# showlab/DiffSim

Measured on AMD Instinct MI355X. Metric: image-pairs/sec at 512px, SD1.5 up_blocks[0] t=600, higher is better.
Workload: dtype bf16

## Files before the change

### diffsim_amd/csrc/common.h

```cpp
#pragma once
#include <hip/hip_runtime.h>
#include <stddef.h>
#include <stdint.h>

#include "../../include/diffsim_amd.h"

namespace dsim {

typedef __bf16 bf16_t;
typedef _Float16 f16_t;
#ifdef DSIM_H16_IS_F16
typedef _Float16 h16;
#define DSIM_H16_NS f16
#define DSIM_H16 DSIM_F16
#define DSIM_H16_ONE_BITS 0x3C00u
#define DSIM_H16_LSUM_MAX 3.0e4f
#define H16_MFMA_16x16x32 __builtin_amdgcn_mfma_f32_16x16x32_f16
#define H16_MFMA_32x32x16 __builtin_amdgcn_mfma_f32_32x32x16_f16
#else
typedef __bf16 h16;
#define DSIM_H16_NS bf16
#define DSIM_H16 DSIM_BF16
#define DSIM_H16_ONE_BITS 0x3F80u
#define DSIM_H16_LSUM_MAX 1e30f
#define H16_MFMA_16x16x32 __builtin_amdgcn_mfma_f32_16x16x32_bf16
#define H16_MFMA_32x32x16 __builtin_amdgcn_mfma_f32_32x32x16_bf16
#endif
typedef __attribute__((ext_vector_type(8))) h16 h16x8;
typedef __attribute__((ext_vector_type(4))) h16 h16x4;
typedef __attribute__((ext_vector_type(2))) h16 h16x2;
typedef __attribute__((ext_vector_type(4))) float f32x4;
typedef __attribute__((ext_vector_type(16))) float f32x16;
typedef __attribute__((ext_vector_type(4))) unsigned int u32x4;
typedef __attribute__((ext_vector_type(2))) unsigned int u32x2;

#ifdef __HIPCC__
__device__ __forceinline__ h16x4 h16_ds_read_tr16_b64(const char* p) {
#ifdef DSIM_H16_IS_F16
    typedef __fp16 fp16v4 __attribute__((__vector_size__(4 * sizeof(__fp16))));
    return __builtin_bit_cast(h16x4, __builtin_amdgcn_ds_read_tr16_b64_v4f16((__attribute__((address_space(3))) fp16v4*)(p)));
#else
    return __builtin_amdgcn_ds_read_tr16_b64_v4bf16((__attribute__((address_space(3))) h16x4*)(p));
#endif
}
__device__ __forceinline__ float gelu_fast(float x) {
    const float u = fminf(x * x, 64.0f);
    const float t = x * fmaf(u, fmaf(u, 1.01426306e-3f, -0.106775724f), -2.30112134f);
    return x * __builtin_amdgcn_rcpf(1.0f + __builtin_amdgcn_exp2f(t));
}
__device__ __forceinline__ float max_halves(float x) {
    const unsigned u = __float_as_uint(x);
    const auto r = __builtin_amdgcn_permlane32_swap(u, u, false, false);
    return fmaxf(__uint_as_float(r[0]), __uint_as_float(r[1]));
}
__device__ __forceinline__ float half_sum(float x) {
    const unsigned u = __float_as_uint(x);
    const auto r = __builtin_amdgcn_permlane32_swap(u, u, false, false);
    return __uint_as_float(r[0]) + __uint_as_float(r[1]);
}
constexpr unsigned BUF_OOB = 0x80000000u;
__device__ __forceinline__ __attribute__((const)) __amdgpu_buffer_rsrc_t buf_rsrc(const void* ptr, unsigned bytes) {
    return __builtin_amdgcn_make_buffer_rsrc((void*)ptr, 0, (int)bytes, 0x00020000);
}
#endif

#define DSIM_HIP_CHECK(expr)                                   \
    do {                                                       \
        hipError_t _e = (expr);                                \
        if (_e != hipSuccess) return DSIM_ERR_HIP;             \
    } while (0)

static inline size_t dtype_size(int dt) { return dt == DSIM_F32 ? 4 : 2; }
static inline const char* dtype_name(int dt) { return dt == DSIM_F32 ? "f32" : (dt == DSIM_F16 ? "f16" : "bf16"); }

template <typename T> struct Elem { typedef T type; };
template <typename F>
int by_dtype(int dtype, F&& f) {
    switch (dtype) {
        case DSIM_BF16: return f(Elem<bf16_t>{});
        case DSIM_F16: return f(Elem<f16_t>{});
        case DSIM_F32: return f(Elem<float>{});
    }
    return DSIM_ERR_INVALID;
}
template <typename F, typename Twin>
int by_h16_dtype(int dtype, F&& f, Twin&& twin) {
    if (dtype == DSIM_H16) return f(Elem<h16>{});
#ifndef DSIM_H16_IS_F16
    if (dtype == DSIM_F32) return f(Elem<float>{});
    if (dtype == DSIM_F16) return twin();
#endif
    return DSIM_ERR_INVALID;
}

static inline size_t up256(size_t bytes) { return (bytes + 255) & ~(size_t)255; }

enum GemmMode { GEMM_LINEAR = 0, GEMM_CONV3 = 1, GEMM_CONV3P = 2 };
enum GemmEpi { EPI_NONE = 0, EPI_RESIDUAL = 1, EPI_GEGLU = 2 };
enum { EK_PLAIN = 0, EK_RES = 1, EK_SLOW = 2, EK_ACT = 3,
       EK_PLAIN_GN = 4, EK_RES_GN = 5 };

struct GemmArgs {
    const void* A0 = nullptr;
    const void* A1 = nullptr;
    int C0 = 0, C1 = 0;
    int mode = GEMM_LINEAR;
    int Hin = 0, Win = 0, Hout = 0, Wout = 0;
    int stride = 1, ups = 0;
    int pad = 1;
    int lwo = -1, lhw = -1;
    int M = 0, N = 0, K = 0;
    const void* W = nullptr;
    const float* bias = nullptr;
    const float* bias2 = nullptr;
    int rows_per_batch = 0;
    int act = 0;
    const float* gate = nullptr;
    const float* gate2 = nullptr;
    int epi = EPI_NONE;
    int geglu_blk = 32;
    const void* residual = nullptr;
    void* out = nullptr;
    int ldo = 0;
    int out_split = 0;
    long long out_split_stride = 0;
    int force_big = 0;
    int wb_rows = 0;
    unsigned wb_stride = 0;
    float* gn_part = nullptr;
    int gn_hw = 0;
    const void* zero_page = nullptr;
    unsigned a0_bytes = 0, a1_bytes = 0, w_bytes = 0, out_bytes = 0;
#ifdef DSIM_DEVTOOLS
    int exp = 0;
    unsigned long long* stamps = nullptr;
#endif
};
struct GemmLaunchRec {
    int bm = 0, bn = 0, mode = -1, geglu = 0, ek = -1, small = 0;
};
extern thread_local GemmLaunchRec g_gemm_last_launch;
inline int geglu_block_rows(int N) { return (N % 320 == 0 && N != 8 * 320) ? 16 : 32; }
#ifdef DSIM_DEVTOOLS
extern int g_gemm_persistent;
extern int g_force_bm;
extern int g_gemm_exp;
extern int g_gemm_skinny;
extern unsigned long long* g_gemm_stamps;
extern int g_skinny_tile;
extern int g_attn_dbg;
extern float* g_tail160_dbg;
extern int g_tail160_exp;
extern int g_ff_dbg;
extern int g_rl_dbg;
extern int g_rl_wpc;
extern int g_ff_stagger;
#else
constexpr int g_gemm_skinny = 1, g_gemm_persistent = 1, g_force_bm = 0, g_gemm_exp = 0, g_skinny_tile = 0;
constexpr int g_rl_wpc = 3, g_ff_stagger = -1;
#endif
constexpr int kSkinnyTiles[][2] = {{64, 64}, {64, 80}, {64, 128}, {128, 80}, {128, 128},
#ifdef DSIM_DEVTOOLS
                                   {128, 64}, {128, 160},
#endif
};
constexpr int kSkinnyChoices = 5, kSkinnyCompiled = sizeof(kSkinnyTiles) / sizeof(kSkinnyTiles[0]);
int pack_linear(const void* src, int src_dtype, void* dst, int dst_dtype, int N, int K,
                int geglu_interleave, hipStream_t s);
int pack_conv3(const void* src, int src_dtype, void* dst, int dst_dtype, int Cout, int Cin,
               hipStream_t s);
int pack_conv_in(const void* src, int src_dtype, float* dst, int Cout, int Cin, hipStream_t s);
int pack_vector(const void* src, int src_dtype, float* dst, int N, int geglu_interleave,
                hipStream_t s);
int gemv_f32(const void* W, int w_dtype, const void* bias, int b_dtype, const float* x, float* y,
             int N, int K, int act, hipStream_t s);
int add_vectors_f32(const float* a, const float* b, float* out, int N, hipStream_t s);
int timestep_sincos(float* out, int dim, int t, hipStream_t s);
int sincos_values(float* out, int dim, const float* vals , int count, hipStream_t s);

int prep_conv_in(const float* lat, const float* noise , float sa, float sb, const float* w ,
                 const float* bias, void* out, int dtype, int n_img, int Cin, int S, int Cout, int dup ,
                 hipStream_t st);
enum { CONV_IN_GENERIC = 1, CONV_IN_EIGHT = 2, CONV_IN_ROWS = 3 };
bool prep_conv_in_kind_applies(int kind, int Cin, int Cout);
int prep_conv_in_kind(int Cin, int Cout);
int prep_conv_in_as(int kind, const float* lat, const float* noise, float sa, float sb, const float* w, const float* bias, void* out,
                    int dtype, int n_img, int Cin, int S, int Cout, int dup, hipStream_t st);
bool conv_in_rows_applies(int Cin, int S, int Cout);
int conv_in_rows(const float* images, const float* w , const float* bias, void* out, int dtype, int n_img, int S,
                 float* gn_part, hipStream_t st);
int convert_f32_to(const float* src, void* dst, int dtype, size_t n, hipStream_t s);
int gather_ctx(const float* ctx, int n_ctx, const int32_t* index, void* dst, int dtype, int n_images, size_t per, hipStream_t s);
int dup_batch(const void* in, void* out, int n_batch, size_t bytes_per_elem, hipStream_t s);
int resize_nearest(const void* in, void* out, int B, int Hin, int Win, int Hout, int Wout, size_t row_bytes, hipStream_t s);

int patch_embed(const float* lat, const float* noise, float sa, float sb, const float* w, const float* bias, const float* pos, void* out,
                int dtype, int n_img, int Cin, int S, int p, int D, hipStream_t s);
int fold_quant(const float* wq, const void* wco, const float* bco, const float* bq, void* out_w, float* out_b, int Cm, int K, int dtype,
               hipStream_t s);
int to_nchw_f32(const void* x, float* out, int n, int HW, int C, int dtype, hipStream_t s);

struct RowLinArgs {
    const void* x = nullptr;
    void* out = nullptr;
    const float* ln_g = nullptr;
    const float* ln_b = nullptr;
    const void* stream = nullptr;
    int M = 0, C = 0, N = 0;
    float eps = 1e-5f;
    int dtype = DSIM_BF16;
    int gn = 0;
    const float* coef = nullptr;
    const float* bias = nullptr;
    int HW = 0;
};

int image_preprocess(const unsigned char* hwc, float* out, int n, int H, int W, int half, hipStream_t s);
int latent_sample(const float* moments, const float* eps, float* out, int n_out, int first, int stride, int C, int hw, int eps_n,
                  float sf, int round16, hipStream_t s);

size_t groupnorm_scratch_bytes(int B, int groups);
int groupnorm_passes(int C0, int C1, int HW, int groups, int dtype);
int groupnorm_plan(int C0, int C1, int B, int HW, int groups, int dtype, int pre, dsim_gn_plan* plan);
int layernorm_plan(int M, int C, int dtype, int mod, dsim_ln_plan* plan);
int launch_groupnorm(const void* x0, int C0, const void* x1, int C1, const float* gamma,
                     const float* beta, void* out, int B, int HW, int groups, float eps, int silu,
                     int dtype, void* scratch, hipStream_t s);
int launch_groupnorm_pre(const void* x, int C, const float* gamma, const float* beta, void* out, int B, int HW, int groups, float eps,
                         int silu, int dtype, void* scratch, const float* part32, int chunks, hipStream_t s);
int launch_groupnorm_stats(const void* x, int C, const float* gamma, const float* beta, int B, int HW, int groups, float eps, int dtype,
                           void* scratch, float* coef, hipStream_t s);
int launch_layernorm(const void* x, const float* gamma, const float* beta, void* out, int M, int C,
                     float eps, int dtype, hipStream_t s);
int launch_layernorm_mod(const void* x, const float* scale2, const float* shift2, void* out, int M, int C,
                         int rows_per_batch, float eps, int dtype, hipStream_t s);
int launch_softmax_rows(const void* x, void* out, int rows, int cols, float scale, int dtype, hipStream_t s);

struct AttnArgs {
    const void* q = nullptr; int ldq = 0;
    const void* k = nullptr; const void* v = nullptr; int ldk = 0;
    void* out = nullptr; int ldo = 0;
    int B = 0, Bkv = 0, H = 0, Nq = 0, Nk = 0, D = 0;
    int xcd_remap = 1;
};
enum class AttnKernel {
    P160 = DSIM_ATTN_P160,
    Short = DSIM_ATTN_SHORT,
    ShortK80 = DSIM_ATTN_SHORT_K80,
    Long = DSIM_ATTN_LONG,
    Q2 = DSIM_ATTN_Q2,
    Q2Fast = DSIM_ATTN_Q2FAST,
    Fast = DSIM_ATTN_FAST,
    Exact = DSIM_ATTN_EXACT,
};
inline const char* attn_kind_suffix(int kind) {
    switch (kind) {
        case DSIM_ATTN_P160: return "_p160";
        case DSIM_ATTN_SHORT:
        case DSIM_ATTN_SHORT_K80: return "_short";
        case DSIM_ATTN_LONG: return "_long";
        case DSIM_ATTN_Q2: return "_q2";
        case DSIM_ATTN_Q2FAST: return "_q2fast";
        case DSIM_ATTN_FAST: return "_fast";
        default: return "";
    }
}
struct AttnLaunchRec {
    int kind = -1, D = 0, dtype = -1, k80 = 0, qit = 0, grid = 0;
};
extern thread_local AttnLaunchRec g_attn_last_launch;
int launch_attention_fp8(const AttnArgs& a, hipStream_t s);

struct PairArgs {
    const void* q = nullptr;
    const void* k = nullptr;
    const void* v = nullptr;
    const int32_t* idx_a = nullptr;
    const int32_t* idx_b = nullptr;
    int n_pairs = 0, B = 0, H = 0, N = 0, D = 0;
    int similarity = 0;
    void* scratch = nullptr;
    size_t scratch_bytes = 0;
};

struct MatrixArgs {
    const void* q[2];
    const void* k[2];
    const void* v[2];
    const uint8_t* mask[2];
    int n_a, n_b, B, H, N, D;
    int similarity;
    void* scratch;
    size_t scratch_bytes;
};

struct FFArgs {
    const void* x = nullptr;
    void* out = nullptr;
    const float* ln_g = nullptr;
    const float* ln_b = nullptr;
    const void* stream = nullptr;
    const float* b1 = nullptr;
    const float* b2 = nullptr;
    int M = 0, C = 0;
    float eps = 1e-5f;
    int dtype = DSIM_BF16;
};

inline namespace DSIM_H16_NS {
#include "h16_api.h"
inline bool gemm_gn_stats_tile(const GemmArgs& a, int dtype) {
    if (dtype == DSIM_F32 || a.mode != GEMM_CONV3 || a.epi == EPI_GEGLU || a.bias2 || a.Wout <= 0) return false;
    const int hw = a.Hout * a.Wout;
    if ((a.Wout & (a.Wout - 1)) || (hw & (hw - 1)) || hw % 256) return false;
    float asked = 0.f;
    GemmArgs q = a;
    q.gn_part = &asked; q.gn_hw = hw; q.zero_page = &asked;
    GemmLaunchRec plan;
    return gemm_plan(q, dtype, &plan) == DSIM_OK;
}
inline int pair_args_check(const PairArgs& a, int dtype, bool tiled = true) {
    if (dtype != DSIM_F32 && dtype != DSIM_BF16 && dtype != DSIM_F16) return DSIM_ERR_INVALID;
    if (a.similarity != 0 && a.similarity != 1) return DSIM_ERR_INVALID;
    return pair_shape_served(a.n_pairs, a.B, a.H, a.N, a.D, tiled) ? DSIM_OK : DSIM_ERR_INVALID;
}
inline int matrix_args_check(const MatrixArgs& a, int dtype, bool listed) {
    if (a.similarity != 0 && a.similarity != 1) return DSIM_ERR_INVALID;
    return matrix_shape_served(a.n_a, a.n_b, a.B, a.H, a.N, a.D, dtype, listed) ? DSIM_OK : DSIM_ERR_INVALID;
}
}
#if !defined(DSIM_H16_IS_F16) && !defined(DSIM_DEVTOOLS)
namespace f16 {
#include "h16_api.h"
}
#define DSIM_F16_TWIN(call) f16::call
#else
#define DSIM_F16_TWIN(call) DSIM_ERR_INVALID
#endif

int cu_count();
struct DeviceOnce {
    unsigned long long done = 0;
    template <typename F> int ensure(F&& apply) {
        int dev = 0;
        if (hipGetDevice(&dev) != hipSuccess) return DSIM_ERR_HIP;
        if (dev >= 0 && dev < 64 && (__atomic_load_n(&done, __ATOMIC_ACQUIRE) >> dev) & 1ull) return DSIM_OK;
        const int st = apply();
        if (st == DSIM_OK && dev >= 0 && dev < 64) __atomic_fetch_or(&done, 1ull << dev, __ATOMIC_RELEASE);
        return st;
    }
};
template <auto Kern, typename... A>
int launch_lds(dim3 grid, dim3 block, int lds_bytes, hipStream_t s, A... args) {
    static DeviceOnce once;
    const int st = once.ensure([&]() -> int {
        return hipFuncSetAttribute((const void*)Kern, hipFuncAttributeMaxDynamicSharedMemorySize, lds_bytes) == hipSuccess ? DSIM_OK
                                                                                                                            : DSIM_ERR_HIP;
    });
    if (st != DSIM_OK) return st;
    hipLaunchKernelGGL(Kern, grid, block, lds_bytes, s, args...);
    return hipGetLastError() == hipSuccess ? DSIM_OK : DSIM_ERR_HIP;
}

}
```

### diffsim_amd/csrc/rowres.hip

```cpp
#include "common.h"

namespace dsim {
namespace {

constexpr int RC = 320;
constexpr int RKS = RC / 16;
constexpr int RNB = RC / 32;
constexpr int RNCH = 4 * RC / 32;
constexpr int RITER = RNCH + 2;
constexpr int RW1B = 64 * RC * 2;
constexpr int RW2B = RC * 64;
constexpr int RCHB = RW1B + RW2B;
constexpr int RPIECES = RCHB / 1024;
constexpr int RPW = RPIECES / 4;
constexpr int RB1 = 0, RB2 = 8 * RC, RLG = 9 * RC, RLB = 10 * RC, RVEC = 11 * RC;
constexpr int SLABP = 144;
constexpr int RSCR = 32 * SLABP;
constexpr int RLDS = 2 * RCHB + RVEC * 4 + 4 * RSCR;
static_assert(RPIECES % 4 == 0 && RITER % 2 == 0, "ring geometry");

__device__ __forceinline__ int slab_chunk(int row, int cpos) { return cpos ^ ((row >> 1) & 7); }
__device__ __forceinline__ int slab_off(int row, int c) { const int s = (row >> 1) & 7; return row * 128 + ((c ^ s) << 4); }
__device__ __forceinline__ u32x4 slab_image(const h16* __restrict__ w, int row0, int slab, int row, int cpos, int ldw = RC, int k0 = 0) {
    const int cl = slab_chunk(row, cpos);
    return *reinterpret_cast<const u32x4*>(w + (size_t)(row0 + row) * ldw + k0 + 64 * slab + 8 * cl);
}

__global__ void pack_ff_stream_kernel(const h16* __restrict__ w1p, const h16* __restrict__ w2p, char* __restrict__ stream) {
    const int i = blockIdx.x * blockDim.x + threadIdx.x;
    if (i >= RITER * (RCHB / 16)) return;
    const int ci = i / (RCHB / 16), o = (i - ci * (RCHB / 16)) * 16;
    u32x4 v = {0u, 0u, 0u, 0u};
    if (o < RW1B) {
        if (ci < RNCH) v = slab_image(w1p, 64 * ci, o / 8192, (o % 8192) / 128, (o % 128) / 16);
    } else {
        if (ci >= 2) {
            const int c = ci - 2, o2 = o - RW1B;
            const int row = o2 / 64, cpos = (o2 % 64) / 16;
            const int cl = cpos ^ ((row >> 2) & 3);
            const int s = cl >> 1, hh = cl & 1;
            h16x8 e;
#pragma unroll
            for (int j = 0; j < 8; ++j)
                e[j] = w2p[(size_t)row * (4 * RC) + 32 * c + 16 * s + 8 * (j >> 2) + 4 * hh + (j & 3)];
            v = __builtin_bit_cast(u32x4, e);
        }
    }
    *reinterpret_cast<u32x4*>(stream + (size_t)ci * RCHB + o) = v;
}

template <int KS>
__device__ __forceinline__ void row_stats(u32x4 (&x)[KS], float eps, float& mean, float& rstd) {
    float sum = 0.f;
#pragma unroll
    for (int ks = 0; ks < KS; ++ks) {
        const h16x8 t = __builtin_bit_cast(h16x8, x[ks]);
#pragma unroll
        for (int j = 0; j < 8; ++j) sum += (float)t[j];
    }
    sum = half_sum(sum);
    mean = sum * (1.0f / (16 * KS));
    float sq = 0.f;
#pragma unroll
    for (int ks = 0; ks < KS; ++ks) {
        asm volatile("" : "+v"(x[ks]));
        const h16x8 t = __builtin_bit_cast(h16x8, x[ks]);
#pragma unroll
        for (int j = 0; j < 8; ++j) { const float d = (float)t[j] - mean; sq = fmaf(d, d, sq); }
    }
    sq = half_sum(sq);
    rstd = 1.0f / sqrtf(sq * (1.0f / (16 * KS)) + eps);
}
__device__ __forceinline__ h16x8 row_norm(u32x4& x, int ks, int half, float mean, float rstd, const float* gamma, const float* beta) {
    const int c = 16 * ks + 8 * half;
    const f32x4 g0 = *reinterpret_cast<const f32x4*>(gamma + c), g1 = *reinterpret_cast<const f32x4*>(gamma + c + 4);
    const f32x4 b0 = *reinterpret_cast<const f32x4*>(beta + c), b1 = *reinterpret_cast<const f32x4*>(beta + c + 4);
    asm volatile("" : "+v"(x));
    const h16x8 t = __builtin_bit_cast(h16x8, x);
    h16x8 y;
#pragma unroll
    for (int j = 0; j < 4; ++j) {
        y[j] = (h16)fmaf(((float)t[j] - mean) * rstd, g0[j], b0[j]);
        y[4 + j] = (h16)fmaf(((float)t[4 + j] - mean) * rstd, g1[j], b1[j]);
    }
    return y;
}
__device__ __forceinline__ void slab_put(char* srow, int bb, int half, const f32x16& a) {
#pragma unroll
    for (int q = 0; q < 4; ++q) {
        h16x4 pk;
#pragma unroll
        for (int e = 0; e < 4; ++e) pk[e] = (h16)a[4 * q + e];
        *reinterpret_cast<h16x4*>(srow + (bb * 32 + 8 * q + 4 * half) * 2) = pk;
    }
}

struct FFParams {
    const h16* x;
    h16* out;
    const float* ln_g;
    const float* ln_b;
    const char* stream;
    const float* b1;
    const float* b2;
    int M;
    float eps;
    unsigned x_bytes, stream_bytes;
    int stagger;
};

template <int DBG>
__global__ __launch_bounds__(256, 1) void ff_fused_kernel(const FFParams p, const int ntiles) {
    extern __shared__ __attribute__((aligned(16))) char smem[];
    const int tid = threadIdx.x, lane = tid & 63, l31 = lane & 31, half = lane >> 5;
    const int wave = __builtin_amdgcn_readfirstlane(tid >> 6);

    const __amdgpu_buffer_rsrc_t rX = buf_rsrc(p.x, p.x_bytes);
    const __amdgpu_buffer_rsrc_t rO = buf_rsrc(p.out, p.x_bytes);
    const __amdgpu_buffer_rsrc_t rS = buf_rsrc(p.stream, p.stream_bytes);

    auto dma = [&](int sp, int ci, int d) {
        if (DBG & 1) return;
        char* dst = smem + sp * RCHB + wave * (RPW * 1024) + d * 1024;
        __builtin_amdgcn_raw_ptr_buffer_load_lds(rS, (__attribute__((address_space(3))) void*)dst, 16, lane * 16,
                                                 ci * RCHB + wave * (RPW * 1024) + d * 1024, 0, 0);
    };
#pragma unroll
    for (int d = 0; d < RPW; ++d) dma(0, 0, d);
    float* const vec = reinterpret_cast<float*>(smem + 2 * RCHB);
    for (int i = tid; i < RVEC / 4; i += 256) {
        const int e = 4 * i;
        const float* src = e < RB2 ? p.b1 + e : (e < RLG ? p.b2 + (e - RB2) : (e < RLB ? p.ln_g + (e - RLG) : p.ln_b + (e - RLB)));
        *reinterpret_cast<f32x4*>(vec + e) = *reinterpret_cast<const f32x4*>(src);
    }

    int w1off[4];
#pragma unroll
    for (int kk = 0; kk < 4; ++kk) w1off[kk] = slab_off(l31, 2 * kk + half);
    const int sw2 = (l31 >> 2) & 3;
    int w2off[2];
#pragma unroll
    for (int s = 0; s < 2; ++s) w2off[s] = RW1B + l31 * 64 + (((2 * s + half) ^ sw2) << 4);

    u32x4 raw[RKS];
    auto load_rows = [&](int tile) {
        const int row = tile * 128 + wave * 32 + l31;
        const unsigned rbase = (tile < ntiles && row < p.M) ? (unsigned)row * (RC * 2) + half * 16 : BUF_OOB;
#pragma unroll
        for (int ks = 0; ks < RKS; ++ks) raw[ks] = __builtin_amdgcn_raw_buffer_load_b128(rX, (int)(rbase + ks * 32), 0, 0);
    };
    load_rows(blockIdx.x);
    __syncthreads();

    for (int tile = blockIdx.x; tile < ntiles; tile += gridDim.x) {
        const int m0 = tile * 128 + wave * 32;
        h16x8 X[RKS];
        {
            float mean, rstd;
            row_stats(raw, p.eps, mean, rstd);
#pragma unroll
            for (int ks = 0; ks < RKS; ++ks) X[ks] = row_norm(raw[ks], ks, half, mean, rstd, vec + RLG, vec + RLB);
        }
        __builtin_amdgcn_sched_barrier(0);
        f32x16 out[RNB];
#pragma unroll
        for (int b = 0; b < RNB; ++b)
#pragma unroll
            for (int q = 0; q < 4; ++q) {
                const f32x4 b4 = *reinterpret_cast<const f32x4*>(vec + RB2 + 32 * b + 8 * q + 4 * half);
#pragma unroll
                for (int e = 0; e < 4; ++e) out[b][4 * q + e] = b4[e];
            }
        __builtin_amdgcn_sched_barrier(0);

        f32x16 aH[2], aG[2];
        h16x8 wf[2][4];
        h16x8 p0, p1;
        h16x8 q0, q1;
        float hv[16];

        auto stagger_wait = [&]() {
            int cnt = wave * p.stagger;
            asm volatile("s_cmp_eq_u32 %0, 0\n\ts_cbranch_scc1 .Lstag_end_%=\n.Lstag_%=:\n\ts_nop 7\n\ts_sub_u32 %0, %0, 1\n\t"
                         "s_cmp_lg_u32 %0, 0\n\ts_cbranch_scc1 .Lstag_%=\n.Lstag_end_%=:" : "+s"(cnt) :: "scc");
        };
        auto init1 = [&](int c, f32x16& h, f32x16& gg) {
#pragma unroll
            for (int q = 0; q < 4; ++q) {
                const f32x4 bh = *reinterpret_cast<const f32x4*>(vec + RB1 + 64 * c + 8 * q + 4 * half);
                const f32x4 bg = *reinterpret_cast<const f32x4*>(vec + RB1 + 64 * c + 32 + 8 * q + 4 * half);
#pragma unroll
                for (int e = 0; e < 4; ++e) { h[4 * q + e] = bh[e]; gg[4 * q + e] = bg[e]; }
            }
        };
        auto ld1 = [&](const char* slot, int i, h16x8 (&w)[4]) {
            if ((DBG & 16) && i > 0) return;
#pragma unroll
            for (int u = 0; u < 2; ++u) {
                const int ks = 2 * i + u;
                const char* a = slot + (ks >> 2) * 8192 + w1off[ks & 3];
                w[2 * u] = *reinterpret_cast<const h16x8*>(a);
                w[2 * u + 1] = *reinterpret_cast<const h16x8*>(a + 32 * 128);
            }
        };
        auto mm1 = [&](int i, const h16x8 (&w)[4], f32x16& h, f32x16& gg) {
#pragma unroll
            for (int u = 0; u < 2; ++u) {
                if (DBG & 4) { asm volatile("" :: "v"(w[2 * u]), "v"(w[2 * u + 1]), "v"(X[2 * i + u])); continue; }
                h = H16_MFMA_32x32x16(w[2 * u], X[2 * i + u], h, 0, 0, 0);
                gg = H16_MFMA_32x32x16(w[2 * u + 1], X[2 * i + u], gg, 0, 0, 0);
            }
        };
        auto ld2 = [&](const char* slot, int j, h16x8 (&w)[4]) {
            if (DBG & 16) return;
#pragma unroll
            for (int u = 0; u < 2; ++u) {
                w[2 * u] = *reinterpret_cast<const h16x8*>(slot + w2off[0] + (2 * j + u) * 2048);
                w[2 * u + 1] = *reinterpret_cast<const h16x8*>(slot + w2off[1] + (2 * j + u) * 2048);
            }
        };
        auto mm2 = [&](int j, const h16x8 (&w)[4]) {
#pragma unroll
            for (int u = 0; u < 2; ++u) {
                if (DBG & 8) { asm volatile("" :: "v"(w[2 * u]), "v"(w[2 * u + 1]), "v"(p0), "v"(p1)); continue; }
                out[2 * j + u] = H16_MFMA_32x32x16(w[2 * u], p0, out[2 * j + u], 0, 0, 0);
                out[2 * j + u] = H16_MFMA_32x32x16(w[2 * u + 1], p1, out[2 * j + u], 0, 0, 0);
            }
        };
        auto geglu1 = [&](int e, const f32x16& h, const f32x16& gg) {
            hv[e] = (DBG & 2) ? h[e] + gg[e] : h[e] * gelu_fast(gg[e]);
            if (e & 1) {
                if (e < 8) { q0[e - 1] = (h16)hv[e - 1]; q0[e] = (h16)hv[e]; }
                else { q1[e - 9] = (h16)hv[e - 1]; q1[e - 8] = (h16)hv[e]; }
            }
        };
#define RR_SB __builtin_amdgcn_sched_barrier(0)
#define RR_MIX(NV)                                                                                                    \
        __builtin_amdgcn_sched_group_barrier(0x008, 1, 0); __builtin_amdgcn_sched_group_barrier(0x020, 1, 0);         \
        __builtin_amdgcn_sched_group_barrier(0x002, NV, 0);                                                           \
        __builtin_amdgcn_sched_group_barrier(0x008, 1, 0); __builtin_amdgcn_sched_group_barrier(0x020, 1, 0);         \
        __builtin_amdgcn_sched_group_barrier(0x002, NV, 0);                                                           \
        __builtin_amdgcn_sched_group_barrier(0x008, 1, 0); __builtin_amdgcn_sched_group_barrier(0x002, NV, 0);        \
        __builtin_amdgcn_sched_group_barrier(0x008, 1, 0); __builtin_amdgcn_sched_group_barrier(0x002, NV, 0);
#define RR_BODY(PAR, C, G1, GL, G2, NEXT_CI)                                                                          \
        {                                                                                                             \
            constexpr int NG = ((G1) ? 10 : 0) + ((G2) ? 5 : 0), NH = NG == 15 ? 12 : (NG == 10 ? 8 : 4);             \
            asm volatile("s_waitcnt vmcnt(0)" ::: "memory");                                                          \
            __syncthreads();                                                                                          \
            stagger_wait();                                                              \
            const char* slot = smem + (PAR) * RCHB;                                                                   \
            if (G1) { init1((C), aH[PAR], aG[PAR]); ld1(slot, 0, wf[0]); } else ld2(slot, 0, wf[0]);                  \
            RR_SB;                                                                                                    \
            _Pragma("unroll") for (int n = 0; n < NG; ++n) {                                                          \
                const int gi = (G1) ? n : n + 10;                               \
                if (n + 1 < NG) { if (gi + 1 < 10) ld1(slot, gi + 1, wf[(n + 1) & 1]); else ld2(slot, gi + 1 - 10, wf[(n + 1) & 1]); } \
                RR_SB;                                                                                                \
                if (gi < 10) mm1(gi, wf[n & 1], aH[PAR], aG[PAR]); else mm2(gi - 10, wf[n & 1]);                      \
                _Pragma("unroll") for (int d = 0; d < RPW; ++d) if ((d * NH) / RPW == n) dma((PAR) ^ 1, (NEXT_CI), d); \
                if (GL) { _Pragma("unroll") for (int e = 0; e < 16; ++e) if ((e * NG) / 16 == n) geglu1(e, aH[(PAR) ^ 1], aG[(PAR) ^ 1]); } \
                RR_MIX(4)                                                                                             \
                RR_SB;                                                                                                \
            }                                                                                                         \
            if (GL) { p0 = q0; p1 = q1; }                                                                             \
        }
        RR_BODY(0, 0, true, false, false, 1)
        RR_BODY(1, 1, true, true, false, 2)
        for (int c = 2; c < RNCH; c += 2) {
            RR_BODY(0, c, true, true, true, c + 1)
            RR_BODY(1, c + 1, true, true, true, c + 2)
        }
        load_rows(tile + (int)gridDim.x);
        RR_BODY(0, RNCH, false, true, true, RNCH + 1)
        RR_BODY(1, RNCH + 1, false, false, true, 0)
#undef RR_BODY
#undef RR_MIX
#undef RR_SB

        char* const slab = smem + 2 * RCHB + RVEC * 4 + wave * RSCR;
        u32x4 res[RNB / 2][4];
#pragma unroll
        for (int pp = 0; pp < RNB / 2; ++pp)
#pragma unroll
            for (int it = 0; it < 4; ++it) {
                const int idx = lane + it * 64, r = idx >> 3, c = idx & 7;
                const unsigned go = (m0 + r) < p.M ? (unsigned)(m0 + r) * (RC * 2) + (unsigned)(pp * 128 + c * 16) : BUF_OOB;
                res[pp][it] = __builtin_amdgcn_raw_buffer_load_b128(rX, (int)go, 0, 0);
            }
#pragma unroll
        for (int pp = 0; pp < RNB / 2; ++pp) {
#pragma unroll
            for (int bb = 0; bb < 2; ++bb) slab_put(slab + l31 * SLABP, bb, half, out[2 * pp + bb]);
#pragma unroll
            for (int it = 0; it < 4; ++it) {
                const int idx = lane + it * 64, r = idx >> 3, c = idx & 7;
                const unsigned go = (m0 + r) < p.M ? (unsigned)(m0 + r) * (RC * 2) + (unsigned)(pp * 128 + c * 16) : BUF_OOB;
                const h16x8 t = *reinterpret_cast<const h16x8*>(slab + r * SLABP + c * 16);
                const h16x8 rr = __builtin_bit_cast(h16x8, res[pp][it]);
                h16x8 o;
#pragma unroll
                for (int e = 0; e < 8; ++e) o[e] = (h16)((float)t[e] + (float)rr[e]);
                __builtin_amdgcn_raw_buffer_store_b128(__builtin_bit_cast(u32x4, o), rO, (int)go, 0, 0);
            }
        }
    }
    asm volatile("s_waitcnt vmcnt(0)" ::: "memory");
}

constexpr int LCHB = 32 * RC * 2;
constexpr int LPW = LCHB / 1024 / 4;
constexpr int LSCR = 16 * SLABP;
constexpr int rowlin_lds(int K, bool GN) { return 2 * LCHB + 2 * K * 4 + (GN ? K * 4 : 0) + 4 * LSCR; }
static_assert(rowlin_lds(RC, false) == 52736, "three workgroups per CU");

__global__ void pack_rowlin_stream_kernel(const h16* __restrict__ wp, char* __restrict__ stream, int N, int K) {
    const int i = blockIdx.x * blockDim.x + threadIdx.x;
    const int kh = K / RC;
    if (i >= N / 32 * kh * (LCHB / 16)) return;
    const int t = i / (LCHB / 16), o = (i - t * (LCHB / 16)) * 16;
    *reinterpret_cast<u32x4*>(stream + (size_t)t * LCHB + o) =
        slab_image(wp, 32 * (t / kh), o / 4096, (o % 4096) / 128, (o % 128) / 16, K, RC * (t % kh));
}

struct RLParams {
    const h16* x;
    h16* out;
    const float* ln_g;
    const float* ln_b;
    const char* stream;
    int M, N;
    float eps;
    unsigned x_bytes, out_bytes, stream_bytes;
    const float* coef;
    const float* bias;
    int HW;
};

template <int K, bool GN, int DBG>
__device__ __forceinline__ void rowlin_body(const RLParams& p, const int ntiles) {
    constexpr int KS = K / 16, KH = K / RC;
    extern __shared__ __attribute__((aligned(16))) char smem[];
    const int tid = threadIdx.x, lane = tid & 63, l31 = lane & 31, half = lane >> 5;
    const int wave = __builtin_amdgcn_readfirstlane(tid >> 6);
    const __amdgpu_buffer_rsrc_t rX = buf_rsrc(p.x, p.x_bytes);
    const __amdgpu_buffer_rsrc_t rO = buf_rsrc(p.out, p.out_bytes);
    const __amdgpu_buffer_rsrc_t rS = buf_rsrc(p.stream, p.stream_bytes);
    const int nblk = p.N / 32 * KH;
    auto dma = [&](int sp, int blk) {
        char* dst = smem + sp * LCHB + wave * (LPW * 1024);
#pragma unroll
        for (int d = 0; d < LPW; ++d)
            __builtin_amdgcn_raw_ptr_buffer_load_lds(rS, (__attribute__((address_space(3))) void*)(dst + d * 1024), 16, lane * 16,
                                                     blk * LCHB + wave * (LPW * 1024) + d * 1024, 0, 0);
    };
    dma(0, 0);
    float* const vec = reinterpret_cast<float*>(smem + 2 * LCHB);
    float* const bvec = vec + 2 * K;
    if (GN) {
        for (int i = tid; i < K; i += 256) bvec[i] = (p.bias && i < p.N) ? p.bias[i] : 0.f;
    } else if (p.ln_g) {
        for (int i = tid; i < 2 * K; i += 256) vec[i] = i < K ? p.ln_g[i] : p.ln_b[i - K];
    }
    char* const slab = smem + rowlin_lds(K, GN) - 4 * LSCR + wave * LSCR;
    int woff[4];
#pragma unroll
    for (int kk = 0; kk < 4; ++kk) woff[kk] = slab_off(l31, 2 * kk + half);
    __syncthreads();
    int blk = 0;

    for (int tile = blockIdx.x; tile < ntiles; tile += gridDim.x) {
        const int m0 = tile * 128 + wave * 32;
        u32x4 xr[KS];
        {
            const int row = m0 + l31;
            const unsigned rbase = row < p.M ? (unsigned)row * (K * 2) + half * 16 : BUF_OOB;
#pragma unroll
            for (int ks = 0; ks < KS; ++ks)
                xr[ks] = (DBG & 4) ? u32x4{(unsigned)ks, 1u, 2u, rbase} : __builtin_amdgcn_raw_buffer_load_b128(rX, (int)(rbase + ks * 32), 0, 0);
            if (GN) {
                if (p.coef) {
                    const float* src = p.coef + (size_t)(tile * 128 / p.HW) * (2 * K);
                    for (int i = tid; i < 2 * K / 4; i += 256)
                        *reinterpret_cast<f32x4*>(vec + 4 * i) = *reinterpret_cast<const f32x4*>(src + 4 * i);
                    __syncthreads();
#pragma unroll
                    for (int ks = 0; ks < KS; ++ks) {
                        const int c = 16 * ks + 8 * half;
                        const f32x4 s0 = *reinterpret_cast<const f32x4*>(vec + c), s1 = *reinterpret_cast<const f32x4*>(vec + c + 4);
                        const f32x4 h0 = *reinterpret_cast<const f32x4*>(vec + K + c), h1 = *reinterpret_cast<const f32x4*>(vec + K + c + 4);
                        const h16x8 t = __builtin_bit_cast(h16x8, xr[ks]);
                        h16x8 y;
#pragma unroll
                        for (int j = 0; j < 4; ++j) {
                            float f0 = fmaf((float)t[j], s0[j], h0[j]), f1 = fmaf((float)t[4 + j], s1[j], h1[j]);
                            asm("" : "+v"(f0), "+v"(f1));
                            y[j] = (h16)f0;
                            y[4 + j] = (h16)f1;
                        }
                        xr[ks] = __builtin_bit_cast(u32x4, y);
                    }
                }
            } else if (p.ln_g) {
                float mean, rstd;
                row_stats(xr, p.eps, mean, rstd);
#pragma unroll
                for (int ks = 0; ks < KS; ++ks) {
                    xr[ks] = __builtin_bit_cast(u32x4, row_norm(xr[ks], ks, half, mean, rstd, vec, vec + K));
                    __builtin_amdgcn_sched_barrier(0);
                }
            }
        }
        __builtin_amdgcn_sched_barrier(0);
        h16x8 wf[2][2];
        auto step = [&](int sp, f32x16& a, int kh, bool stored, int col) {
            if (stored) asm volatile("s_waitcnt vmcnt(4)" ::: "memory");
            else asm volatile("s_waitcnt vmcnt(0)" ::: "memory");
            __syncthreads();
            const int nb = blk + 1 == nblk ? 0 : blk + 1;
            dma(sp ^ 1, nb);
            blk = nb;
            const char* slot = smem + sp * LCHB;
            if (kh == 0) {
                if (GN) {
#pragma unroll
                    for (int q = 0; q < 4; ++q) {
                        const f32x4 b4 = *reinterpret_cast<const f32x4*>(bvec + col + 8 * q + 4 * half);
#pragma unroll
                        for (int e = 0; e < 4; ++e) a[4 * q + e] = b4[e];
                    }
                } else {
#pragma unroll
                    for (int e = 0; e < 16; ++e) a[e] = 0.f;
                }
            }
            auto ld = [&](int i, h16x8 (&w)[2]) {
#pragma unroll
                for (int u = 0; u < 2; ++u) {
                    const int ks = 2 * i + u;
                    w[u] = *reinterpret_cast<const h16x8*>(slot + (ks >> 2) * 4096 + woff[ks & 3]);
                }
            };
            ld(0, wf[0]);
            __builtin_amdgcn_sched_barrier(0);
#pragma unroll
            for (int i = 0; i < 10; ++i) {
                if (i < 9 && !(DBG & 8)) ld(i + 1, wf[(i + 1) & 1]);
                __builtin_amdgcn_sched_barrier(0);
#pragma unroll
                for (int u = 0; u < 2; ++u)
                    if (!(DBG & 2)) a = H16_MFMA_32x32x16(wf[i & 1][u], __builtin_bit_cast(h16x8, xr[RKS * kh + 2 * i + u]), a, 0, 0, 0);
                __builtin_amdgcn_sched_barrier(0);
            }
        };
        auto store_pair = [&](const f32x16& a0, const f32x16& a1, int col0) {
#pragma unroll
            for (int ph = 0; ph < 2; ++ph) {
                asm volatile("" ::: "memory");
                if ((l31 >> 4) == ph) {
#pragma unroll
                    for (int bb = 0; bb < 2; ++bb) slab_put(slab + (l31 & 15) * SLABP, bb, half, bb ? a1 : a0);
                }
#pragma unroll
                for (int it = 0; it < 2; ++it) {
                    const int idx = lane + it * 64, r = idx >> 3, c = idx & 7, row = m0 + 16 * ph + r;
                    const unsigned go = row < p.M ? ((unsigned)row * (unsigned)p.N + (unsigned)col0) * 2u + (unsigned)c * 16u : BUF_OOB;
                    const u32x4 t = *reinterpret_cast<const u32x4*>(slab + r * SLABP + c * 16);
                    if (!(DBG & 1) || t[0] == 0x12345u) __builtin_amdgcn_raw_buffer_store_b128(t, rO, (int)go, 0, 0);
                }
            }
        };
        f32x16 a0, a1;
        for (int pr = 0; pr < p.N / 64; ++pr) {
            if (KH == 1) {
                step(0, a0, 0, true, 64 * pr);
                step(1, a1, 0, false, 64 * pr + 32);
            } else {
                step(0, a0, 0, true, 64 * pr);
                step(1, a0, 1, false, 64 * pr);
                step(0, a1, 0, false, 64 * pr + 32);
                step(1, a1, 1, false, 64 * pr + 32);
            }
            store_pair(a0, a1, 64 * pr);
        }
    }
    asm volatile("s_waitcnt vmcnt(0)" ::: "memory");
}

template <int DBG>
__global__ __launch_bounds__(256, 3) void rowlin_kernel(const RLParams p, const int ntiles) { rowlin_body<RC, false, DBG>(p, ntiles); }
template <int DBG>
__global__ __launch_bounds__(256, 2) void rowlin640_kernel(const RLParams p, const int ntiles) { rowlin_body<2 * RC, false, DBG>(p, ntiles); }
template <int K, int DBG>
__global__ __launch_bounds__(256, K == RC ? 3 : 2) void gn_rowlin_kernel(const RLParams p, const int ntiles) { rowlin_body<K, true, DBG>(p, ntiles); }

template <auto Kern, typename P>
int launch_rows(const P& p, int wpc, int lds, hipStream_t s) {
    const int ntiles = (p.M + 127) / 128, cap = wpc * cu_count();
    return launch_lds<Kern>(dim3(ntiles < cap ? ntiles : cap), dim3(256), lds, s, p, ntiles);
}

}

#ifdef DSIM_DEVTOOLS
int g_rl_dbg = 0;
int g_ff_dbg = 0;
int g_ff_stagger = -1;
int g_rl_wpc = 3;
#endif

inline namespace DSIM_H16_NS {
size_t ff_stream_bytes(int C) { return C == RC ? (size_t)RITER * RCHB : 0; }

int pack_ff_stream(const void* w1_packed, const void* w2_packed, void* stream, int C, hipStream_t s) {
    if (C != RC) return DSIM_ERR_INVALID;
    const int n = RITER * (RCHB / 16);
    hipLaunchKernelGGL(pack_ff_stream_kernel, dim3((n + 255) / 256), dim3(256), 0, s, (const h16*)w1_packed,
                       (const h16*)w2_packed, (char*)stream);
    DSIM_HIP_CHECK(hipGetLastError());
    return DSIM_OK;
}

int launch_ff_fused(const FFArgs& a, hipStream_t s) {
    if (a.dtype != DSIM_H16) return a.dtype == DSIM_F16 ? DSIM_F16_TWIN(launch_ff_fused(a, s)) : DSIM_ERR_INVALID;
    if (a.C != RC || a.M < 1 || (size_t)a.M * RC * 2 >= 0x7fffffffull) return DSIM_ERR_INVALID;
    FFParams p;
    p.x = (const h16*)a.x; p.out = (h16*)a.out; p.ln_g = a.ln_g; p.ln_b = a.ln_b; p.stream = (const char*)a.stream;
    p.b1 = a.b1; p.b2 = a.b2; p.M = a.M; p.eps = a.eps;
    p.x_bytes = (unsigned)((size_t)a.M * RC * 2);
    p.stream_bytes = (unsigned)((size_t)RITER * RCHB);
    p.stagger = g_ff_stagger >= 0 ? g_ff_stagger : 1;
#ifdef DSIM_DEVTOOLS
    switch (g_ff_dbg) {
#define X(d) case d: return launch_rows<ff_fused_kernel<d>>(p, 1, RLDS, s);
        X(1) X(2) X(3) X(12) X(13) X(15) X(16) X(31)
#undef X
        default: break;
    }
#endif
    return launch_rows<ff_fused_kernel<0>>(p, 1, RLDS, s);
}

size_t rowlin_stream_bytes(int C, int N) {
    return ((C == RC || C == 2 * RC) && N >= 64 && N % 64 == 0 && N <= 3 * C) ? (size_t)N / 32 * (C / RC) * LCHB : 0;
}

int pack_rowlin_stream(const void* w_packed, void* stream, int C, int N, hipStream_t s) {
    if (!rowlin_stream_bytes(C, N)) return DSIM_ERR_INVALID;
    const int n = N / 32 * (C / RC) * (LCHB / 16);
    hipLaunchKernelGGL(pack_rowlin_stream_kernel, dim3((n + 255) / 256), dim3(256), 0, s, (const h16*)w_packed, (char*)stream, N, C);
    DSIM_HIP_CHECK(hipGetLastError());
    return DSIM_OK;
}

int launch_rowlin(const RowLinArgs& a, hipStream_t s) {
    if (a.dtype != DSIM_H16) return a.dtype == DSIM_F16 ? DSIM_F16_TWIN(launch_rowlin(a, s)) : DSIM_ERR_INVALID;
    if (!rowlin_stream_bytes(a.C, a.N) || a.M < 1 || (size_t)a.M * a.N * 2 >= 0x7fffffffull || (size_t)a.M * a.C * 2 >= 0x7fffffffull ||
        !a.ln_g != !a.ln_b) return DSIM_ERR_INVALID;
    if (a.gn && (a.ln_g || a.N > a.C || (a.coef && (a.HW < 128 || a.HW % 128 || a.M % a.HW)))) return DSIM_ERR_INVALID;
    if (!a.gn && (a.coef || a.bias)) return DSIM_ERR_INVALID;
    RLParams p;
    p.x = (const h16*)a.x; p.out = (h16*)a.out; p.ln_g = a.ln_g; p.ln_b = a.ln_b; p.stream = (const char*)a.stream;
    p.M = a.M; p.N = a.N; p.eps = a.eps;
    p.x_bytes = (unsigned)((size_t)a.M * a.C * 2); p.out_bytes = (unsigned)((size_t)a.M * a.N * 2);
    p.stream_bytes = (unsigned)rowlin_stream_bytes(a.C, a.N);
    p.coef = a.coef; p.bias = a.bias; p.HW = a.HW > 0 ? a.HW : 1;
    if (a.gn)
        return a.C == RC ? launch_rows<gn_rowlin_kernel<RC, 0>>(p, 3, rowlin_lds(RC, true), s)
                         : launch_rows<gn_rowlin_kernel<2 * RC, 0>>(p, 2, rowlin_lds(2 * RC, true), s);
    if (a.C != RC) return launch_rows<rowlin640_kernel<0>>(p, 2, rowlin_lds(2 * RC, false), s);
#ifdef DSIM_DEVTOOLS
    switch (g_rl_dbg) {
#define X(d) case d: return launch_rows<rowlin_kernel<d>>(p, g_rl_wpc, rowlin_lds(RC, false), s);
        X(1) X(2) X(4) X(8) X(10) X(15)
#undef X
        default: break;
    }
#endif
    return launch_rows<rowlin_kernel<0>>(p, g_rl_wpc, rowlin_lds(RC, false), s);
}
}

}
```

Measured before the change: 688.0.

## Process two 128-row blocks per streamed weight chunk in rowlin for wide N

Adds a ROWS=2 variant of the row-linear kernel that holds two 128-row blocks of activations in registers and reuses each streamed weight chunk for both, halving weight streaming per output row. It is selected by default for non-GN layers with N >= 960 at K=320, launched at two workgroups per CU. The store path is restructured to pack the first half-tile to h16 registers before the second step. The cost is doubled row registers and lower occupancy.

```diff
diff --git a/diffsim_amd/csrc/common.h b/diffsim_amd/csrc/common.h
--- a/diffsim_amd/csrc/common.h
+++ b/diffsim_amd/csrc/common.h
@@ -154,10 +154,11 @@
 extern int g_ff_dbg;
 extern int g_rl_dbg;
 extern int g_rl_wpc;
+extern int g_rl_rows;
 extern int g_ff_stagger;
 #else
 constexpr int g_gemm_skinny = 1, g_gemm_persistent = 1, g_force_bm = 0, g_gemm_exp = 0, g_skinny_tile = 0;
-constexpr int g_rl_wpc = 3, g_ff_stagger = -1;
+constexpr int g_rl_wpc = 0, g_rl_rows = 0, g_ff_stagger = -1;
 #endif
 constexpr int kSkinnyTiles[][2] = {{64, 64}, {64, 80}, {64, 128}, {128, 80}, {128, 128},
 #ifdef DSIM_DEVTOOLS
diff --git a/diffsim_amd/csrc/rowres.hip b/diffsim_amd/csrc/rowres.hip
--- a/diffsim_amd/csrc/rowres.hip
+++ b/diffsim_amd/csrc/rowres.hip
@@ -309,8 +309,10 @@
 constexpr int LCHB = 32 * RC * 2;
 constexpr int LPW = LCHB / 1024 / 4;
 constexpr int LSCR = 16 * SLABP;
-constexpr int rowlin_lds(int K, bool GN) { return 2 * LCHB + 2 * K * 4 + (GN ? K * 4 : 0) + 4 * LSCR; }
-static_assert(rowlin_lds(RC, false) == 52736, "three workgroups per CU");
+constexpr int rowlin_rows(bool gn, int N) { return !gn && N >= 3 * RC ? 2 : 1; }
+constexpr int rowlin_lds(int K, bool GN, int ROWS = 1) { return 2 * LCHB + (GN ? ROWS : 1) * 2 * K * 4 + (GN ? K * 4 : 0) + 4 * LSCR; }
+static_assert(rowlin_lds(RC, false) == 52736 && 3 * rowlin_lds(RC, true) <= 160 * 1024, "ROWS = 1 at K = 320: three workgroups per CU");
+static_assert(2 * rowlin_lds(RC, true, 2) <= 160 * 1024 && 2 * rowlin_lds(2 * RC, true) <= 160 * 1024, "two workgroups per CU");
 
 __global__ void pack_rowlin_stream_kernel(const h16* __restrict__ wp, char* __restrict__ stream, int N, int K) {
     const int i = blockIdx.x * blockDim.x + threadIdx.x;
@@ -335,9 +337,11 @@
     int HW;
 };
 
-template <int K, bool GN, int DBG>
+template <int K, bool GN, int DBG, int ROWS = 1>
 __device__ __forceinline__ void rowlin_body(const RLParams& p, const int ntiles) {
+    static_assert(ROWS == 1 || (ROWS == 2 && K == RC), "two row blocks are 160 registers of rows at K = 320; 320 at K = 640");
     constexpr int KS = K / 16, KH = K / RC;
+    constexpr int TR = 128 * ROWS;
     extern __shared__ __attribute__((aligned(16))) char smem[];
     const int tid = threadIdx.x, lane = tid & 63, l31 = lane & 31, half = lane >> 5;
     const int wave = __builtin_amdgcn_readfirstlane(tid >> 6);
@@ -354,13 +358,13 @@
     };
     dma(0, 0);
     float* const vec = reinterpret_cast<float*>(smem + 2 * LCHB);
-    float* const bvec = vec + 2 * K;
+    float* const bvec = vec + (GN ? ROWS : 1) * 2 * K;
     if (GN) {
         for (int i = tid; i < K; i += 256) bvec[i] = (p.bias && i < p.N) ? p.bias[i] : 0.f;
     } else if (p.ln_g) {
         for (int i = tid; i < 2 * K; i += 256) vec[i] = i < K ? p.ln_g[i] : p.ln_b[i - K];
     }
-    char* const slab = smem + rowlin_lds(K, GN) - 4 * LSCR + wave * LSCR;
+    char* const slab = smem + rowlin_lds(K, GN, ROWS) - 4 * LSCR + wave * LSCR;
     int woff[4];
 #pragma unroll
     for (int kk = 0; kk < 4; ++kk) woff[kk] = slab_off(l31, 2 * kk + half);
@@ -368,52 +372,68 @@
     int blk = 0;
 
     for (int tile = blockIdx.x; tile < ntiles; tile += gridDim.x) {
-        const int m0 = tile * 128 + wave * 32;
-        u32x4 xr[KS];
+        const int m0 = tile * TR + wave * 32;
+        u32x4 xr[ROWS][KS];
         {
-            const int row = m0 + l31;
-            const unsigned rbase = row < p.M ? (unsigned)row * (K * 2) + half * 16 : BUF_OOB;
-#pragma unroll
-            for (int ks = 0; ks < KS; ++ks)
-                xr[ks] = (DBG & 4) ? u32x4{(unsigned)ks, 1u, 2u, rbase} : __builtin_amdgcn_raw_buffer_load_b128(rX, (int)(rbase + ks * 32), 0, 0);
+#pragma unroll
+            for (int q = 0; q < ROWS; ++q) {
+                const int row = m0 + 128 * q + l31;
+                const unsigned rbase = row < p.M ? (unsigned)row * (K * 2) + half * 16 : BUF_OOB;
+#pragma unroll
+                for (int ks = 0; ks < KS; ++ks)
+                    xr[q][ks] = (DBG & 4) ? u32x4{(unsigned)ks, 1u, 2u, rbase} : __builtin_amdgcn_raw_buffer_load_b128(rX, (int)(rbase + ks * 32), 0, 0);
+            }
             if (GN) {
                 if (p.coef) {
-                    const float* src = p.coef + (size_t)(tile * 128 / p.HW) * (2 * K);
-                    for (int i = tid; i < 2 * K / 4; i += 256)
-                        *reinterpret_cast<f32x4*>(vec + 4 * i) = *reinterpret_cast<const f32x4*>(src + 4 * i);
+                    for (int i = tid; i < ROWS * (2 * K / 4); i += 256) {
+                        const int q = ROWS == 1 ? 0 : i / (2 * K / 4);
+                        int r0 = tile * TR + 128 * q;
+                        if (ROWS > 1 && r0 >= p.M) r0 = p.M - 1;
+                        const float* src = p.coef + (size_t)(r0 / p.HW) * (2 * K);
+                        *reinterpret_cast<f32x4*>(vec + 4 * i) = *reinterpret_cast<const f32x4*>(src + 4 * (i - q * (2 * K / 4)));
+                    }
                     __syncthreads();
 #pragma unroll
-                    for (int ks = 0; ks < KS; ++ks) {
-                        const int c = 16 * ks + 8 * half;
-                        const f32x4 s0 = *reinterpret_cast<const f32x4*>(vec + c), s1 = *reinterpret_cast<const f32x4*>(vec + c + 4);
-                        const f32x4 h0 = *reinterpret_cast<const f32x4*>(vec + K + c), h1 = *reinterpret_cast<const f32x4*>(vec + K + c + 4);
-                        const h16x8 t = __builtin_bit_cast(h16x8, xr[ks]);
-                        h16x8 y;
-#pragma unroll
-                        for (int j = 0; j < 4; ++j) {
-                            float f0 = fmaf((float)t[j], s0[j], h0[j]), f1 = fmaf((float)t[4 + j], s1[j], h1[j]);
-                            asm("" : "+v"(f0), "+v"(f1));
-                            y[j] = (h16)f0;
-                            y[4 + j] = (h16)f1;
+                    for (int q = 0; q < ROWS; ++q) {
+                        const float* const cf = vec + q * 2 * K;
+#pragma unroll
+                        for (int ks = 0; ks < KS; ++ks) {
+                            const int c = 16 * ks + 8 * half;
+                            const f32x4 s0 = *reinterpret_cast<const f32x4*>(cf + c), s1 = *reinterpret_cast<const f32x4*>(cf + c + 4);
+                            const f32x4 h0 = *reinterpret_cast<const f32x4*>(cf + K + c), h1 = *reinterpret_cast<const f32x4*>(cf + K + c + 4);
+                            const h16x8 t = __builtin_bit_cast(h16x8, xr[q][ks]);
+                            h16x8 y;
+#pragma unroll
+                            for (int j = 0; j < 4; ++j) {
+                                float f0 = fmaf((float)t[j], s0[j], h0[j]), f1 = fmaf((float)t[4 + j], s1[j], h1[j]);
+                                asm("" : "+v"(f0), "+v"(f1));
+                                y[j] = (h16)f0;
+                                y[4 + j] = (h16)f1;
+                            }
+                            xr[q][ks] = __builtin_bit_cast(u32x4, y);
                         }
-                        xr[ks] = __builtin_bit_cast(u32x4, y);
                     }
                 }
             } else if (p.ln_g) {
-                float mean, rstd;
-                row_stats(xr, p.eps, mean, rstd);
-#pragma unroll
-                for (int ks = 0; ks < KS; ++ks) {
-                    xr[ks] = __builtin_bit_cast(u32x4, row_norm(xr[ks], ks, half, mean, rstd, vec, vec + K));
-                    __builtin_amdgcn_sched_barrier(0);
+#pragma unroll
+                for (int q = 0; q < ROWS; ++q) {
+                    float mean, rstd;
+                    row_stats(xr[q], p.eps, mean, rstd);
+#pragma unroll
+                    for (int ks = 0; ks < KS; ++ks) {
+                        xr[q][ks] = __builtin_bit_cast(u32x4, row_norm(xr[q][ks], ks, half, mean, rstd, vec, vec + K));
+                        __builtin_amdgcn_sched_barrier(0);
+                    }
                 }
             }
         }
         __builtin_amdgcn_sched_barrier(0);
         h16x8 wf[2][2];
-        auto step = [&](int sp, f32x16& a, int kh, bool stored, int col) {
-            if (stored) asm volatile("s_waitcnt vmcnt(4)" ::: "memory");
-            else asm volatile("s_waitcnt vmcnt(0)" ::: "memory");
+        auto step = [&](int sp, f32x16 (&a)[ROWS], int kh, bool stored, int col) {
+            if (stored && !(DBG & 1)) {
+                if (ROWS == 1) asm volatile("s_waitcnt vmcnt(4)" ::: "memory");
+                else asm volatile("s_waitcnt vmcnt(8)" ::: "memory");
+            } else asm volatile("s_waitcnt vmcnt(0)" ::: "memory");
             __syncthreads();
             const int nb = blk + 1 == nblk ? 0 : blk + 1;
             dma(sp ^ 1, nb);
@@ -425,11 +445,15 @@
                     for (int q = 0; q < 4; ++q) {
                         const f32x4 b4 = *reinterpret_cast<const f32x4*>(bvec + col + 8 * q + 4 * half);
 #pragma unroll
-                        for (int e = 0; e < 4; ++e) a[4 * q + e] = b4[e];
+                        for (int rb = 0; rb < ROWS; ++rb)
+#pragma unroll
+                            for (int e = 0; e < 4; ++e) a[rb][4 * q + e] = b4[e];
                     }
                 } else {
 #pragma unroll
-                    for (int e = 0; e < 16; ++e) a[e] = 0.f;
+                    for (int rb = 0; rb < ROWS; ++rb)
+#pragma unroll
+                        for (int e = 0; e < 16; ++e) a[rb][e] = 0.f;
                 }
             }
             auto ld = [&](int i, h16x8 (&w)[2]) {
@@ -447,29 +471,49 @@
                 __builtin_amdgcn_sched_barrier(0);
 #pragma unroll
                 for (int u = 0; u < 2; ++u)
-                    if (!(DBG & 2)) a = H16_MFMA_32x32x16(wf[i & 1][u], __builtin_bit_cast(h16x8, xr[RKS * kh + 2 * i + u]), a, 0, 0, 0);
+#pragma unroll
+                    for (int rb = 0; rb < ROWS; ++rb)
+                        if (!(DBG & 2))
+                            a[rb] = H16_MFMA_32x32x16(wf[i & 1][u], __builtin_bit_cast(h16x8, xr[rb][RKS * kh + 2 * i + u]), a[rb], 0, 0, 0);
                 __builtin_amdgcn_sched_barrier(0);
             }
         };
-        auto store_pair = [&](const f32x16& a0, const f32x16& a1, int col0) {
-#pragma unroll
-            for (int ph = 0; ph < 2; ++ph) {
+        auto store_pair = [&](auto&& put, int col0) {
+#pragma unroll
+            for (int rp = 0; rp < 2 * ROWS; ++rp) {
+                const int rb = rp >> 1, ph = rp & 1;
                 asm volatile("" ::: "memory");
-                if ((l31 >> 4) == ph) {
-#pragma unroll
-                    for (int bb = 0; bb < 2; ++bb) slab_put(slab + (l31 & 15) * SLABP, bb, half, bb ? a1 : a0);
-                }
+                if ((l31 >> 4) == ph) put(rb, slab + (l31 & 15) * SLABP);
 #pragma unroll
                 for (int it = 0; it < 2; ++it) {
-                    const int idx = lane + it * 64, r = idx >> 3, c = idx & 7, row = m0 + 16 * ph + r;
+                    const int idx = lane + it * 64, r = idx >> 3, c = idx & 7, row = m0 + 128 * rb + 16 * ph + r;
                     const unsigned go = row < p.M ? ((unsigned)row * (unsigned)p.N + (unsigned)col0) * 2u + (unsigned)c * 16u : BUF_OOB;
                     const u32x4 t = *reinterpret_cast<const u32x4*>(slab + r * SLABP + c * 16);
                     if (!(DBG & 1) || t[0] == 0x12345u) __builtin_amdgcn_raw_buffer_store_b128(t, rO, (int)go, 0, 0);
                 }
             }
         };
-        f32x16 a0, a1;
+        f32x16 a0[ROWS], a1[ROWS];
         for (int pr = 0; pr < p.N / 64; ++pr) {
+            if (ROWS == 2) {
+                h16x4 lo[ROWS][4];
+                step(0, a0, 0, true, 64 * pr);
+#pragma unroll
+                for (int rb = 0; rb < ROWS; ++rb)
+#pragma unroll
+                    for (int q = 0; q < 4; ++q) {
+#pragma unroll
+                        for (int e = 0; e < 4; ++e) lo[rb][q][e] = (h16)a0[rb][4 * q + e];
+                        asm volatile("" : "+v"(lo[rb][q]));
+                    }
+                step(1, a0, 0, false, 64 * pr + 32);
+                store_pair([&](int rb, char* srow) {
+#pragma unroll
+                    for (int q = 0; q < 4; ++q) *reinterpret_cast<h16x4*>(srow + (8 * q + 4 * half) * 2) = lo[rb][q];
+                    slab_put(srow, 1, half, a0[rb]);
+                }, 64 * pr);
+                continue;
+            }
             if (KH == 1) {
                 step(0, a0, 0, true, 64 * pr);
                 step(1, a1, 0, false, 64 * pr + 32);
@@ -479,22 +523,27 @@
                 step(0, a1, 0, false, 64 * pr + 32);
                 step(1, a1, 1, false, 64 * pr + 32);
             }
-            store_pair(a0, a1, 64 * pr);
+            store_pair([&](int rb, char* srow) {
+#pragma unroll
+                for (int bb = 0; bb < 2; ++bb) slab_put(srow, bb, half, bb ? a1[rb] : a0[rb]);
+            }, 64 * pr);
         }
     }
     asm volatile("s_waitcnt vmcnt(0)" ::: "memory");
 }
 
 template <int DBG>
-__global__ __launch_bounds__(256, 3) void rowlin_kernel(const RLParams p, const int ntiles) { rowlin_body<RC, false, DBG>(p, ntiles); }
+__global__ __launch_bounds__(256, 3) void rowlin_kernel(const RLParams p, const int ntiles) { rowlin_body<RC, false, DBG, 1>(p, ntiles); }
+template <int DBG>
+__global__ __launch_bounds__(256, 2) void rowlin2_kernel(const RLParams p, const int ntiles) { rowlin_body<RC, false, DBG, 2>(p, ntiles); }
 template <int DBG>
 __global__ __launch_bounds__(256, 2) void rowlin640_kernel(const RLParams p, const int ntiles) { rowlin_body<2 * RC, false, DBG>(p, ntiles); }
-template <int K, int DBG>
-__global__ __launch_bounds__(256, K == RC ? 3 : 2) void gn_rowlin_kernel(const RLParams p, const int ntiles) { rowlin_body<K, true, DBG>(p, ntiles); }
+template <int K, int DBG, int ROWS>
+__global__ __launch_bounds__(256, K == RC && ROWS == 1 ? 3 : 2) void gn_rowlin_kernel(const RLParams p, const int ntiles) { rowlin_body<K, true, DBG, ROWS>(p, ntiles); }
 
 template <auto Kern, typename P>
-int launch_rows(const P& p, int wpc, int lds, hipStream_t s) {
-    const int ntiles = (p.M + 127) / 128, cap = wpc * cu_count();
+int launch_rows(const P& p, int wpc, int lds, hipStream_t s, int rows = 128) {
+    const int ntiles = (p.M + rows - 1) / rows, cap = wpc * cu_count();
     return launch_lds<Kern>(dim3(ntiles < cap ? ntiles : cap), dim3(256), lds, s, p, ntiles);
 }
 
@@ -504,7 +553,8 @@
 int g_rl_dbg = 0;
 int g_ff_dbg = 0;
 int g_ff_stagger = -1;
-int g_rl_wpc = 3;
+int g_rl_wpc = 0;
+int g_rl_rows = 0;
 #endif
 
 inline namespace DSIM_H16_NS {
@@ -563,20 +613,29 @@
     p.x_bytes = (unsigned)((size_t)a.M * a.C * 2); p.out_bytes = (unsigned)((size_t)a.M * a.N * 2);
     p.stream_bytes = (unsigned)rowlin_stream_bytes(a.C, a.N);
     p.coef = a.coef; p.bias = a.bias; p.HW = a.HW > 0 ? a.HW : 1;
-    if (a.gn)
-        return a.C == RC ? launch_rows<gn_rowlin_kernel<RC, 0>>(p, 3, rowlin_lds(RC, true), s)
-                         : launch_rows<gn_rowlin_kernel<2 * RC, 0>>(p, 2, rowlin_lds(2 * RC, true), s);
-    if (a.C != RC) return launch_rows<rowlin640_kernel<0>>(p, 2, rowlin_lds(2 * RC, false), s);
+    if (a.C != RC)
+        return a.gn ? launch_rows<gn_rowlin_kernel<2 * RC, 0, 1>>(p, 2, rowlin_lds(2 * RC, true), s)
+                    : launch_rows<rowlin640_kernel<0>>(p, 2, rowlin_lds(2 * RC, false), s);
+    const int rows = g_rl_rows ? g_rl_rows : rowlin_rows(a.gn, a.N);
+    const int wpc = g_rl_wpc ? g_rl_wpc : (rows == 2 ? 2 : 3);
+    if (a.gn) {
+#ifdef DSIM_DEVTOOLS
+        if (rows == 2) return launch_rows<gn_rowlin_kernel<RC, 0, 2>>(p, wpc, rowlin_lds(RC, true, 2), s, 256);
+#endif
+        return launch_rows<gn_rowlin_kernel<RC, 0, 1>>(p, wpc, rowlin_lds(RC, true), s);
+    }
 #ifdef DSIM_DEVTOOLS
     switch (g_rl_dbg) {
-#define X(d) case d: return launch_rows<rowlin_kernel<d>>(p, g_rl_wpc, rowlin_lds(RC, false), s);
+#define X(d) case d: return rows == 2 ? launch_rows<rowlin2_kernel<d>>(p, wpc, rowlin_lds(RC, false), s, 256) \
+                                      : launch_rows<rowlin_kernel<d>>(p, wpc, rowlin_lds(RC, false), s);
         X(1) X(2) X(4) X(8) X(10) X(15)
 #undef X
         default: break;
     }
 #endif
-    return launch_rows<rowlin_kernel<0>>(p, g_rl_wpc, rowlin_lds(RC, false), s);
-}
-}
-
-}
+    return rows == 2 ? launch_rows<rowlin2_kernel<0>>(p, wpc, rowlin_lds(RC, false), s, 256)
+                     : launch_rows<rowlin_kernel<0>>(p, wpc, rowlin_lds(RC, false), s);
+}
+}
+
+}
```

New measurement: 688.6 (median of 2 runs). No clear change (+0.1%).
